# matchylabs/matchy

Hardware: AMD Instinct MI355X
Metric: log GB/s scanned (matchy match hot path, 100K IoCs) (higher is better)
Workload: dtype u8

## Files before the change

matchy_amd/csrc/device_common.h:

```cpp
#pragma once
#include <hip/hip_runtime.h>

#include "domain_prefilter.h"
#include "hashes.h"
#include "scan_types.h"

namespace mxy {

constexpr uint32_t C_B = 1, C_DIG = 2, C_DOT = 4, C_COLON = 8, C_AT = 16, C_LD = 32, C_NL = 64, C_TLD1 = 128;

constexpr uint64_t bnd_lo() {
    uint64_t m = 0;
    const int cs[] = {0x09, 0x0a, 0x0d, 0x20, 0x22, 0x27, 0x28, 0x29, 0x2c, 0x2f, 0x3a, 0x3b, 0x3c, 0x3d, 0x3e};
    for (int c : cs) m |= 1ull << c;
    return m;
}
constexpr uint64_t bnd_hi() {
    uint64_t m = 0;
    const int cs[] = {0x40, 0x5b, 0x5d, 0x7b, 0x7d};
    for (int c : cs) m |= 1ull << (c - 64);
    return m;
}
__device__ __forceinline__ bool d_is_boundary(uint32_t b) {
    if (b >= 128) return false;
    uint64_t m = b < 64 ? bnd_lo() : bnd_hi();
    return (m >> (b & 63)) & 1;
}
__device__ __forceinline__ bool d_is_digit(uint32_t b) { return b - '0' < 10u; }
__device__ __forceinline__ bool d_is_alpha(uint32_t b) { return (b | 0x20) - 'a' < 26u; }
__device__ __forceinline__ bool d_is_alnum(uint32_t b) { return d_is_digit(b) || d_is_alpha(b); }
__device__ __forceinline__ bool d_is_hex(uint32_t b) { return d_is_digit(b) || ((b | 0x20) - 'a' < 6u); }
__device__ __forceinline__ bool d_is_domain_char_fast(uint32_t b) { return d_is_alnum(b) || b == '-' || b == '.' || b >= 0x80; }
__device__ __forceinline__ bool d_is_domain_char(uint32_t b) { return d_is_alnum(b) || b == '-' || b == '.'; }
__device__ __forceinline__ bool d_is_email_local(uint32_t b) { return d_is_alnum(b) || b == '.' || b == '-' || b == '_' || b == '+'; }

__device__ __forceinline__ uint32_t class_of(uint32_t b) {
    uint32_t c = 0;
    if (d_is_boundary(b)) c |= C_B;
    if (d_is_digit(b)) c |= C_DIG;
    if (b == '.') c |= C_DOT;
    if (b == ':') c |= C_COLON;
    if (b == '@') c |= C_AT;
    if (d_is_alnum(b) || b >= 0x80) c |= C_LD;
    if (b == '\n') c |= C_NL;
    return c;
}

__device__ __forceinline__ uint32_t lane_id() { return __lane_id(); }
__device__ __forceinline__ uint64_t lanemask_lt() { return (1ull << lane_id()) - 1ull; }
__device__ __forceinline__ uint32_t mbcnt64_add(uint64_t m, uint32_t base) {
    return __builtin_amdgcn_mbcnt_hi((uint32_t)(m >> 32), __builtin_amdgcn_mbcnt_lo((uint32_t)m, base));
}
__device__ __forceinline__ uint32_t mbcnt64(uint64_t m) {
    return __builtin_amdgcn_mbcnt_hi((uint32_t)(m >> 32), __builtin_amdgcn_mbcnt_lo((uint32_t)m, 0u));
}

template <class T, uint32_t CHUNK>
struct ChunkWriter {
    static_assert(CHUNK >= 64, "one append can carry 64 entries");
    uint32_t base = 0xFFFFFFFFu;
    uint32_t used = 0;
    uint32_t total = 0;

    __device__ __forceinline__ void pad_rest(T* out, uint32_t cap, const T& sentinel) {
        if (base == 0xFFFFFFFFu) return;
        for (uint32_t k = used + lane_id(); k < CHUNK; k += 64)
            if (base + k < cap) out[base + k] = sentinel;
        used = CHUNK;
    }
    __device__ __forceinline__ void append(bool emit, const T& v, T* out, uint32_t cap, uint32_t* counter, const T& sentinel) {
        const uint64_t m = __ballot(emit);
        if (m == 0) return;
        const uint32_t n = (uint32_t)__popcll(m);
        if (base == 0xFFFFFFFFu || used + n > CHUNK) {
            pad_rest(out, cap, sentinel);
            uint32_t b = 0;
            if (lane_id() == 0) b = atomicAdd(counter, CHUNK);
            base = __builtin_amdgcn_readfirstlane(b);
            used = 0;
        }
        if (emit) {
            const uint32_t slot = base + used + (uint32_t)__popcll(m & lanemask_lt());
            if (slot < cap) out[slot] = v;
        }
        used += n;
        total += n;
    }
};

template <class T> __device__ __forceinline__ T list_sentinel();
template <> __device__ __forceinline__ Candidate list_sentinel<Candidate>() { return Candidate{0u, 0xFFFFFFFFu, 0u, 0u}; }
template <> __device__ __forceinline__ RareAnchor list_sentinel<RareAnchor>() { return RareAnchor{0xFFFFFFFFu, 0xFFu}; }
template <> __device__ __forceinline__ uint32_t list_sentinel<uint32_t>() { return 0xFFFFFFFFu; }
template <> __device__ __forceinline__ uint2 list_sentinel<uint2>() { return make_uint2(0xFFFFFFFFu, 0xFFu); }

template <class T, uint32_t CAP = 64>
struct BufferedWriter {
    T* buf;
    uint32_t cnt = 0;
    uint32_t total = 0;
    uint32_t base = 0xFFFFFFFFu, used = 0, ccap = 0, flushes = 0;
    __device__ __forceinline__ explicit BufferedWriter(T* lds) : buf(lds) {}
    __device__ __forceinline__ void pad_rest(T* out, uint32_t cap) {
        if (base == 0xFFFFFFFFu) return;
        for (uint32_t k = used + lane_id(); k < ccap; k += 64) if (base + k < cap) out[base + k] = list_sentinel<T>();
        used = ccap;
    }
// ... 285 lines not shown
```

matchy_amd/csrc/engine.cpp:

```cpp
#include "engine.h"
#include "batch_reader.h"
#include "distinct.h"
#include "extract_render_core.h"
#include "render_core.h"
#include "tally.h"
#include "unicode_lower.h"

#include <dlfcn.h>

#include <algorithm>
#include <chrono>
#include <cstdio>
#include <cstdlib>
#include <cstring>
#include <stdexcept>
#include <unordered_set>

#include "domain_prefilter.h"
#include "hashes.h"

namespace mxy {

void check_launch(const char* kernel) {
    const hipError_t e = hipGetLastError();
// ... 375 lines not shown
        for (const CpRange& r : lt.ignorable) ri.push_back(make_uint2(r.first, r.last));
        for (const CpRange& r : lt.cased) rc.push_back(make_uint2(r.first, r.last));
        lc_map.upload(m); lc_ign.upload(ri); lc_cased.upload(rc);
        view.lc_map = lc_map.p; view.lc_n = (uint32_t)lt.map.size();
        view.lc_ign = lc_ign.p; view.lc_n_ign = (uint32_t)ri.size();
        view.lc_cased = lc_cased.p; view.lc_n_cased = (uint32_t)rc.size();
        bytes_uploaded += m.size() * 4 + (ri.size() + rc.size()) * 8;
    }
    {
        std::vector<uint32_t> lo, go;
        if (img.has_literal) {
            if (!img.lit_data_offsets.empty()) lo = img.lit_data_offsets;
            else {
                uint32_t mx = 0;
                for (auto& kv : img.lit_data_map) mx = std::max(mx, kv.first + 1);
                lo.assign(mx, 0xFFFFFFFFu);
                for (auto& kv : img.lit_data_map) lo[kv.first] = kv.second;
            }
        }
        if (img.has_glob) {
            go.resize(img.pdm_count);
            if (img.pdm_count) memcpy(go.data(), img.bytes.data() + img.pdm_off, img.pdm_count * 4);
        }
        if (lo.empty()) lo.push_back(0xFFFFFFFFu);
        if (go.empty()) go.push_back(0);
        n_lit_offsets = img.has_literal ? (uint32_t)lo.size() : 0;
        n_glob_offsets = img.has_glob ? (uint32_t)img.pdm_count : 0;
        lit_offsets.upload(lo);
        glob_offsets.upload(go);
    }
    psl_slots.upload(psl.slots);
    psl_pool.upload(psl.pool);
    bloom.upload(psl.bloom);
    view.psl_slots = psl_slots.p; view.psl_mask = psl.mask; view.psl_pool = psl_pool.p; view.tld_bloom = bloom.p;
    view.max_tld_len = psl.max_tld_len;
    view.max_suffix_len = psl.max_suffix_len;
    tld_tab.upload(psl.tld_tab);
    view.tld_tab = tld_tab.p;
    tld_pfx.upload(psl.tld_pfx);
    view.tld_pfx = tld_pfx.p;
    for (int k = 0; k < 8; ++k) view.tld_first[k] = psl.tld_first[k];
    bytes_uploaded += psl.slots.size() * sizeof(PslSlot) + psl.pool.size() + psl.bloom.size() * 4;
}

Scanner::Scanner(std::shared_ptr<const DbImage> img, std::shared_ptr<DeviceDb> ddb, uint32_t extract_flags, uint32_t min_labels)
    : img_(std::move(img)), ddb_(std::move(ddb)), flags_(extract_flags), min_labels_(min_labels ? min_labels : 2) {
    MXY_HIP(hipSetDevice(ddb_->device));
    hipDeviceProp_t prop;
    MXY_HIP(hipGetDeviceProperties(&prop, ddb_->device));
    n_cu_ = prop.multiProcessorCount > 0 ? prop.multiProcessorCount : 256;
    counters_.alloc(MAX_SLICES);
    MXY_HIP(hipMemset(counters_.p, 0, sizeof(ScanCounters) * MAX_SLICES));
    counters_clean_ = true;
    host_slices_.alloc(MAX_SLICES);
    for (Event& e : ev_) e.create();
    ev_fork_.create(hipEventDisableTiming);
    ev_join_.create(hipEventDisableTiming);
    aux_stream_.create(hipStreamNonBlocking);
    ev_join2_.create(hipEventDisableTiming);
    aux2_stream_.create(hipStreamNonBlocking);
}

Scanner::~Scanner() = default;

void Scanner::set_unique(bool on) {
    if (on && !distinct_) {
        distinct_ = std::make_unique<DistinctSet>();
        if (getenv("MATCHY_AMD_TRACE")) { distinct_->set_profile(true); profile_ = true; }
    }
    unique_ = on;
}
void Scanner::reset_unique() {
    if (!distinct_) return;
    MXY_HIP(hipSetDevice(ddb_->device));
    distinct_->reset();
}
uint64_t Scanner::unique_count() const { return distinct_ ? distinct_->count() : 0; }

void Scanner::set_tally(bool on) {
    if (on && !tally_) tally_ = std::make_unique<HitTally>();
    tally_on_ = on;
}
void Scanner::reset_tally() {
    if (!tally_) return;
    MXY_HIP(hipSetDevice(ddb_->device));
    tally_->reset();
}
void Scanner::tally_top(size_t limit, std::vector<TallyEntry>& out) {
    out.clear();
    if (!tally_) return;
    MXY_HIP(hipSetDevice(ddb_->device));
    tally_->top(limit, out, nullptr);
}

void Scanner::Work::ensure(uint32_t len) {
    const size_t want_c = std::max<size_t>(4096, (size_t)len / 24);
    const size_t want_r = std::max<size_t>(1024, (size_t)len / 256);
    const size_t want_h = std::max<size_t>(1024, want_c / 4);
    if (cands.n < want_c) cands.alloc(want_c);
    if (hits.n < want_h) hits.alloc(want_h);
    if (ids.n < want_h) ids.alloc(want_h);
    if (cands_a.n < want_c) cands_a.alloc(want_c);
    if (cands_m.n < want_c / 8) cands_m.alloc(want_c / 8);
    if (cands_r.n < want_r) cands_r.alloc(want_r);
    if (cands_d.n < want_r) cands_d.alloc(want_r);
    if (rare.n < want_r) rare.alloc(want_r);
    if (rare_dom.n < want_r) rare_dom.alloc(want_r);
// ... 1207 lines not shown
```

matchy_amd/csrc/k_anchor.hip:

```cpp
#include "anchor_planes.h"
#include "device_shared.h"

namespace mxy {

constexpr int AW = 4;
constexpr int PRIO_BULK = 0, PRIO_CHAIN = 1, PRIO_DRAIN = 2;
constexpr uint32_t BLK_BYTES = AB_BLOCK;
constexpr uint32_t QCAP = 128;
constexpr uint32_t RAW_BYTES = 8192;
static_assert(SEG_ALIGN % RAW_BYTES == 0 && RAW_BYTES % BLK_BYTES == 0 && RAW_BYTES >= 3 * BLK_BYTES, "window wraps on block edges inside a segment");

constexpr uint32_t RAW_MIRROR = 64;
template <int N>
__device__ __forceinline__ void raw_read(const uint32_t* raw32, uint32_t a, uint32_t (&out)[N]) {
    static_assert(4 * (N + 1) <= RAW_MIRROR + 4, "read runs past the mirrored bytes");
    const uint32_t* q = raw32 + ((a & (RAW_BYTES - 1)) >> 2);
    const uint32_t sh = a & 3;
    uint32_t w[N + 1];
#pragma unroll
    for (int i = 0; i <= N; ++i) w[i] = q[i];
#pragma unroll
    for (int i = 0; i < N; ++i) out[i] = __builtin_amdgcn_alignbyte(w[i + 1], w[i], sh);
}

// ... 635 lines not shown
                    uint32_t cleft = cand;
                    while (__ballot(cleft != 0)) {
                        const bool mine = cleft != 0;
                        const uint32_t q = mine ? (uint32_t)__builtin_ctz(cleft) : 0u;
                        cleft &= cleft - 1;
                        const uint64_t Zq = (uint64_t)(uint32_t)__builtin_amdgcn_ds_bpermute((int)(4 * (q + 1)), zt) |
                                            ((uint64_t)(uint32_t)__builtin_amdgcn_ds_bpermute((int)(4 * (q + 17)), zt) << 32);
                        const uint64_t Zprev_row = (uint64_t)(uint32_t)__builtin_amdgcn_ds_bpermute((int)(4 * q), zt) |
                                                   ((uint64_t)(uint32_t)__builtin_amdgcn_ds_bpermute((int)(4 * (q + 16)), zt) << 32);
                        const uint64_t below = lane ? (Zq << (64 - lane)) : 0ull;
                        uint32_t run = lane ? (uint32_t)__clzll((long long)~below) : 0u;
                        run = min(run, lane);
                        bool too_long = false;
                        if (run == lane) {
                            const uint32_t r2 = ~Zprev_row ? (uint32_t)__clzll((long long)~Zprev_row) : 64u;
                            too_long = r2 == 64u;
                            run += r2;
                        }
                        const int32_t it = (int32_t)(64 * q + lane) - (int32_t)run - 1;
                        const uint32_t src_lane = (uint32_t)it & 63u;
                        const uint32_t wb_cur = (uint32_t)__shfl((int)Bcur, (int)src_lane);
                        const uint32_t wb_prev = (uint32_t)__shfl((int)Bprev, (int)src_lane);
                        const uint32_t rowbits = it >= 0 ? ((wb_cur >> (it >> 6)) & 0x01010101u) : ((wb_prev >> 7) & 0x01010101u);
                        const uint32_t hb = rowbits ? (31u - (uint32_t)__clz((int)rowbits)) >> 3 : 0u;
                        const int32_t s = (int32_t)blk + 4 * it + (int32_t)hb + 1;
                        const uint32_t mybits = (Bcur >> q) & 0x01010101u;
                        const uint32_t b0 = mybits ? ((uint32_t)__ffs((int)mybits) - 1u) >> 3 : 0u;
                        const uint32_t e = blk + AB_ROW_BYTES * q + lane_off + b0;
                        const uint32_t tl = e - (uint32_t)s;
                        const bool tok = mine && !too_long && rowbits != 0 &&
                                         ((tl >= 26 && tl <= 62) || tl == 64 || (tl >= 90 && tl <= 110) || tl == 128);
                        cw_tok.append(tok, make_uint2((uint32_t)s, (uint32_t)RARE_TOK | (tl << 8)));
                    }
                    tok_quiet = 0;
                } else if (tok_dense && ++tok_quiet >= TOK_DENSE_HOLD) {
                    tok_dense = false;
                }
                Bprev = Bcur;
            }
        }
        if (dt != dh) drain_dom(rdom, dh, dt, dt - dh, true, cx, cw_dom);
        if (v4t != v4h) drain_v4<INL>(rv4, v4h, v4t, v4t - v4h, true, cx, pend, cw_cand, vl);
    }
    commit_v4<INL>(pend, cx, cw_cand, vl);
    if constexpr (INL) v4_lookup_flush(vl);
    cw_misc.finish();
    cw_tok.finish();
    if (cw_dom.next == 0xFFFFFFFFu && cold_tok()->dom_static) {
        cw_dom.next = (blockIdx.x * 4u + (threadIdx.x >> 6)) * cold_tok()->dom_static;
        cw_dom.left = cold_tok()->dom_static;
    }
    cw_dom.pad_rest(p.dom_list, p.dom_cap);
    cw_cand.finish(p.cands_a, p.cand_a_cap, &p.counters->n_cand_a, Candidate{0u, 0xFFFFFFFFu, 0u, 0u});
    {
        uint32_t nv = pend.n_valid;
#pragma unroll
        for (int off = 32; off > 0; off >>= 1) nv += __shfl_down(nv, off);
        if (lane == 0 && nv) atomicAdd(&cold_tok()->counters->cand_true, nv);
    }
    unsigned long long lines = nl_count;
#pragma unroll
    for (int off = 32; off > 0; off >>= 1) lines += __shfl_down(lines, off);
    if (lane == 0 && lines) atomicAdd(&cold_tok()->counters->lines, lines);
}

int anchor_blocks_per_cu() {
    int n = 0;
    const hipError_t e = hipOccupancyMaxActiveBlocksPerMultiprocessor(&n, k_anchor<true, true>, AW * 64, 0);
    if (e != hipSuccess || n < 1) n = 3;
    return n;
}

void launch_anchor(const TokParams& p, const DevDb& db, int grid, hipStream_t stream) {
    const bool all = (p.flags & EX_ALL) == EX_ALL && !anchor_tl_wide(db);
    if (all && p.inline_v4) hipLaunchKernelGGL((k_anchor<true, true>), dim3(grid), dim3(AW * 64), 0, stream, p, db);
    else if (all) hipLaunchKernelGGL((k_anchor<true, false>), dim3(grid), dim3(AW * 64), 0, stream, p, db);
    else if (p.inline_v4) hipLaunchKernelGGL((k_anchor<false, true>), dim3(grid), dim3(AW * 64), 0, stream, p, db);
    else hipLaunchKernelGGL((k_anchor<false, false>), dim3(grid), dim3(AW * 64), 0, stream, p, db);
    check_launch("launch_anchor");
}

}
```

matchy_amd/csrc/lookup_kernels.hip:

```cpp
#include <hip/hip_runtime.h>

#include <cstdlib>

#include "hashes.h"
#include "scan_types.h"

#include "device_shared.h"

namespace mxy {


__device__ __forceinline__ uint32_t d_utf8_decode(const uint8_t* s, uint32_t& cp) {
    const uint32_t c = s[0];
    if (c < 0x80) { cp = c; return 1; }
    if (c < 0xE0) { cp = ((c & 0x1Fu) << 6) | (s[1] & 0x3Fu); return 2; }
    if (c < 0xF0) { cp = ((c & 0x0Fu) << 12) | ((s[1] & 0x3Fu) << 6) | (s[2] & 0x3Fu); return 3; }
    cp = ((c & 0x07u) << 18) | ((s[1] & 0x3Fu) << 12) | ((s[2] & 0x3Fu) << 6) | (s[3] & 0x3Fu);
    return 4;
}
__device__ bool d_cp_in_ranges(const uint2* r, uint32_t n, uint32_t cp) {
    uint32_t lo = 0, hi = n;
    while (lo < hi) { const uint32_t mid = (lo + hi) >> 1; if (r[mid].y < cp) lo = mid + 1; else hi = mid; }
    return lo < n && r[lo].x <= cp;
}
// ... 540 lines not shown
            uint32_t type = c.len_type >> 24, tl = c.len_type & 0xFFFFFF;
            const uint8_t* text = p.log + c.start;
            h.cand = i; h.start = c.start; h.len_type = c.len_type;
            if (type == IT_IPV4) {
                uint32_t off, pfx;
                if (db.has_ip && trie_v4(db, c.v4, off, pfx)) { h.kind = 2; h.a = off; h.prefix_len = (uint8_t)pfx; emit = true; }
            } else if (type == IT_IPV6) {
                uint16_t seg[8];
                uint32_t off, pfx;
                if (db.has_ip && d_parse_ipv6(text, tl, seg) && trie_v6(db, seg, off, pfx)) { h.kind = 2; h.a = off; h.prefix_len = (uint8_t)pfx; emit = true; }
            } else {
                const bool alnum_tok = type == IT_MD5 || type == IT_SHA1 || type == IT_SHA256 || type == IT_SHA384 || type == IT_SHA512 ||
                                       type == IT_BITCOIN || type == IT_ETHEREUM || type == IT_MONERO;
                if (!db.ac_alnum && alnum_tok) c.pad = CAND_NO_GLOB;
                if (!GLOB && p.ac_filter && p.early_glob && c.pad == CAND_GLOB) {
                } else if (!GLOB && p.ac_filter && (c.pad == CAND_GLOB || (c.pad != CAND_NO_GLOB && (defer_unwalked || ac_touches_output(db, dv, text, tl))))) defer = true;
                else {
                    uint32_t pid = 0xFFFFFFFFu;
                    if (db.has_literal) { uint32_t q; if (lit_lookup(db, text, tl, q)) pid = q; }
                    if constexpr (GLOB) {
                        GlobSetList rs{globs};
                        StarStackFixed stk;
                        glob_find_all(db, dv, text_stage(p.log, p.len, c.start, tl, twin + threadIdx.x * GLOB_WIN_WORDS), outq + threadIdx.x * GLOB_OUTQ, rs, stk);
                        ng = rs.n;
                        spill = rs.over;
                    }
                    if (!spill && (pid != 0xFFFFFFFFu || ng)) { h.kind = 3; h.a = pid; h.n_globs = (uint16_t)ng; emit = true; }
                }
            }
        }
        if (p.direct && !GLOB) {
            if (emit) { pend[pn] = PendRec{h.start, h.len_type, h.a, (uint32_t)h.kind | ((uint32_t)h.prefix_len << 8)}; ++pn; }
            if (__ballot(pn == PEND_RECS)) { pack_pending(p.pk, pn, pend); pn = 0; }
        } else if (p.direct) {
            pack_record(p.pk, emit, h, GLOB ? globs : nullptr);
        } else {
            if (GLOB && emit && ng) {
                uint32_t io = atomicAdd(&p.counters->n_ids, ng);
                h.ids_off = io;
                for (uint32_t k = 0; k < ng; ++k) if (io + k < p.ids_cap) p.ids[io + k] = globs[k];
            }
            cw.append(emit, h, p.hits, p.hit_cap, &p.counters->n_hits, SH);
        }
        if (!GLOB && p.ac_filter) ww.append(defer, i, p.glob_work, p.glob_work_cap, &p.counters->n_glob_work);
        if (GLOB && spill) {
            const uint32_t q = atomicAdd(&p.counters->n_spill, 1u);
            if (q < p.spill_cap) p.spill[q] = i | (p.spill_tag << 31);
        }
    }
    __shared__ uint32_t wg_slots[12];
    if (p.direct && !GLOB) pack_pending<PEND_RECS, true>(p.pk, pn, pend, wg_slots);
    cw.pad_rest(p.hits, p.hit_cap, SH);
    if (!GLOB && p.ac_filter) ww.flush(p.glob_work, p.glob_work_cap, &p.counters->n_glob_work);
    if (lane_id() == 0 && cw.total) atomicAdd(&p.counters->hits_true, cw.total);
    if (p.arrive_chain) {
        __syncthreads();
        if (threadIdx.x == 0) {
            __threadfence_system();
            if (atomicAdd(&p.arrive->arrive_wgs[p.arrive_chain - 1], 1u) == gridDim.x - 1) atomicAdd(&p.arrive->chains_done, 1u);
        }
    }
}

constexpr int SPILL_THREADS = 64;
__global__ __launch_bounds__(SPILL_THREADS) void k_lookup_spill(LookupParams p, DevDb db) {
    __shared__ uint8_t cls[256];
    __shared__ uint32_t rows[DFA_LDS_ENTRIES_GLOB];
    __shared__ uint64_t twin[SPILL_THREADS * GLOB_WIN_WORDS];
    __shared__ uint32_t outq[SPILL_THREADS * GLOB_OUTQ];
    const DfaView dv = dfa_stage<DFA_LDS_ENTRIES_GLOB>(db, cls, rows);
    __syncthreads();
    const uint32_t n = min(p.counters->n_spill, p.spill_cap);
    const uint32_t stride = gridDim.x * blockDim.x, tid = blockIdx.x * blockDim.x + threadIdx.x;
    const uint32_t bit_words = (db.pattern_count + 31) / 32;
    uint32_t* bits = p.spill_scratch + (size_t)tid * p.spill_words;
    ChunkWriter<Hit, HIT_CHUNK> cw;
    Hit SH{};
    SH.kind = 0xFF;
    for (uint32_t base = blockIdx.x * blockDim.x; base < n; base += stride) {
        const uint32_t k = base + threadIdx.x;
        Hit h{};
        bool emit = false;
        if (k < n) {
            const uint32_t tagged = p.spill[k], i = tagged & 0x7FFFFFFFu;
            const bool alt = (tagged >> 31) != 0;
            const Candidate c = alt ? (p.cands_alt && i < p.cand_alt_cap ? p.cands_alt[i] : Candidate{0, 0xFFFFFFFFu, 0, 0})
                                    : (i < p.cand_cap ? p.cands[i] : Candidate{0, 0xFFFFFFFFu, 0, 0});
            if (c.len_type != 0xFFFFFFFFu) {
                const uint32_t tl = c.len_type & 0xFFFFFF;
                h.cand = i; h.start = c.start; h.len_type = c.len_type;
                uint32_t pid = 0xFFFFFFFFu;
                if (db.has_literal) { uint32_t q; if (lit_lookup(db, p.log + c.start, tl, q)) pid = q; }
                for (uint32_t w = 0; w < bit_words; ++w) bits[w] = 0;
                GlobSetBitmap rs{bits, db.pattern_count};
                StarStackMem stk{bits + bit_words, (p.spill_words - bit_words) / 2};
                glob_find_all(db, dv, text_stage(p.log, p.len, c.start, tl, twin + threadIdx.x * GLOB_WIN_WORDS), outq + threadIdx.x * GLOB_OUTQ, rs, stk);
                uint32_t ng = rs.n;
                if (rs.over || ng > 0xFFFFu) { atomicOr(&p.counters->error, 1u); ng = 0; }
                if (ng) {
                    const uint32_t io = atomicAdd(&p.counters->n_ids, ng);
                    h.ids_off = io;
                    uint32_t o = io;
                    for (uint32_t w = 0; w < bit_words; ++w)
                        for (uint32_t m = bits[w]; m; m &= m - 1, ++o)
                            if (o < p.ids_cap) p.ids[o] = 32 * w + (uint32_t)__builtin_ctz(m);
                }
                if (pid != 0xFFFFFFFFu || ng) { h.kind = 3; h.a = pid; h.n_globs = (uint16_t)ng; emit = true; }
            }
        }
        if (p.direct) pack_record(p.pk, emit, h, nullptr);
        else cw.append(emit, h, p.hits, p.hit_cap, &p.counters->n_hits, SH);
    }
    cw.pad_rest(p.hits, p.hit_cap, SH);
    if (lane_id() == 0 && cw.total) atomicAdd(&p.counters->hits_true, cw.total);
}

template <uint32_t NREC>
__global__ __launch_bounds__(256) void k_lookup_ip(LookupParams p, DevDb db) {
    __shared__ __attribute__((aligned(16))) PendRec pend_lds[256 * NREC];
    PendRec* pend = pend_lds + threadIdx.x * NREC;
    uint32_t pn = 0;
    const uint32_t n = min(*p.n_in, p.cand_cap);
    const uint32_t stride = gridDim.x * blockDim.x;
    for (uint32_t base = blockIdx.x * blockDim.x; base < n; base += stride) {
        const uint32_t i = base + threadIdx.x;
        Candidate c{0, 0xFFFFFFFFu, 0, 0};
        if (i < n) c = p.cands[i];
        if (c.len_type != 0xFFFFFFFFu && (c.len_type >> 24) == IT_IPV4) {
            uint32_t off, pfx;
            if (db.has_ip && trie_v4(db, c.v4, off, pfx)) { pend[pn] = PendRec{c.start, c.len_type, off, 2u | (pfx << 8)}; ++pn; }
        }
        if (__ballot(pn == NREC)) { pack_pending<NREC>(p.pk, pn, pend); pn = 0; }
    }
    __shared__ uint32_t wg_slots[12];
    pack_pending<NREC, true>(p.pk, pn, pend, wg_slots);
}
void launch_lookup_ip(const LookupParams& p, const DevDb& db, int grid, bool dense, hipStream_t stream) {
    if (dense) hipLaunchKernelGGL(k_lookup_ip<8>, dim3(grid), dim3(256), 0, stream, p, db);
    else hipLaunchKernelGGL(k_lookup_ip<2>, dim3(grid), dim3(256), 0, stream, p, db);
    check_launch("launch_lookup_ip");
}
void launch_lookup(const LookupParams& p_in, const DevDb& db, int grid, hipStream_t stream) {
    LookupParams p = p_in;
    p.ac_filter = 0; p.from_work = 0;
    const size_t lean_lds = db.dfa ? (size_t)DFA_LDS_ENTRIES * 4 : 0;
    if (!db.has_glob) {
        hipLaunchKernelGGL(k_lookup<false>, dim3(grid), dim3(256), lean_lds, stream, p, db);
    } else if (db.dfa && db.wild_count == 0 && p.glob_work && grid > 1) {
        p.ac_filter = 1;
        const uint32_t arrive_chain = p.arrive_chain;
        p.arrive_chain = 0;
        hipLaunchKernelGGL(k_lookup<false>, dim3(grid), dim3(256), lean_lds, stream, p, db);
        p.arrive_chain = arrive_chain;
        p.ac_filter = 0; p.from_work = 1;
        hipLaunchKernelGGL(k_lookup<true>, dim3(grid), dim3(256), 0, stream, p, db);
    } else {
        hipLaunchKernelGGL(k_lookup<true>, dim3(grid), dim3(256), 0, stream, p, db);
    }
    check_launch("launch_lookup");
}
void launch_lookup_early_glob(const LookupParams& p_in, const DevDb& db, int grid, hipStream_t stream) {
    LookupParams p = p_in;
    p.ac_filter = 0; p.from_work = 1;
    hipLaunchKernelGGL(k_lookup<true>, dim3(grid), dim3(256), 0, stream, p, db);
    check_launch("launch_lookup_early_glob");
}
__global__ __launch_bounds__(256) void k_finish(ScanCounters* dev, ScanCounters* host, uint32_t n_words, uint32_t expect_chains, unsigned long long poll_ticks,
                                                uint32_t next_n_dom) {
    uint32_t* d = reinterpret_cast<uint32_t*>(dev);
    uint32_t* h = reinterpret_cast<uint32_t*>(host);
    __shared__ uint32_t gave_up;
    if (threadIdx.x == 0) gave_up = 0;
    if (expect_chains) {
        if (threadIdx.x == 0) {
            const unsigned long long t0 = wall_clock64();
            if (poll_ticks == 0) gave_up = 1;
            else while (__hip_atomic_load(&dev->chains_done, __ATOMIC_ACQUIRE, __HIP_MEMORY_SCOPE_AGENT) < expect_chains) {
                if (wall_clock64() - t0 > poll_ticks) { gave_up = 1; break; }
                __builtin_amdgcn_s_sleep(8);
            }
        }
        __syncthreads();
        __threadfence();
    } else {
        __syncthreads();
    }
    const bool keep = gave_up != 0;
    for (uint32_t i = threadIdx.x; i < n_words; i += blockDim.x) {
        h[i] = d[i];
        if (!keep) d[i] = 0;
    }
    __syncthreads();
    if (!keep && threadIdx.x == 0 && next_n_dom) dev->n_dom = next_n_dom;
    if (keep && threadIdx.x == 0) host->error |= 8u;
    __threadfence_system();
}
void launch_finish(ScanCounters* dev, ScanCounters* host_pinned, int n_blocks, uint32_t expect_chains, uint32_t next_n_dom, hipStream_t stream) {
    static const unsigned long long poll_ticks = getenv("MATCHY_AMD_FINISH_POLL_US") ? strtoull(getenv("MATCHY_AMD_FINISH_POLL_US"), nullptr, 10) * 100ull : 200000000ull;
    hipLaunchKernelGGL(k_finish, dim3(1), dim3(256), 0, stream, dev, host_pinned, (uint32_t)(n_blocks * sizeof(ScanCounters) / 4), expect_chains, poll_ticks, next_n_dom);
    check_launch("launch_finish");
}
void launch_lookup_spill(const LookupParams& p, const DevDb& db, hipStream_t stream) {
    hipLaunchKernelGGL(k_lookup_spill, dim3(p.spill_blocks), dim3(SPILL_THREADS), 0, stream, p, db);
    check_launch("launch_lookup_spill");
}
uint32_t spill_threads() { return SPILL_THREADS; }

}
```

matchy_amd/csrc/scan_types.h:

```cpp
#pragma once
#include <hip/hip_runtime.h>

#include <cstdint>

namespace mxy {

enum ItemType : uint8_t {
    IT_DOMAIN = 0, IT_EMAIL = 1, IT_IPV4 = 2, IT_IPV6 = 3, IT_MD5 = 4, IT_SHA1 = 5, IT_SHA256 = 6,
    IT_SHA384 = 7, IT_SHA512 = 8, IT_BITCOIN = 9, IT_ETHEREUM = 10, IT_MONERO = 11, IT_COUNT = 12
};
enum ExtractFlags : uint32_t {
    EX_DOMAINS = 1, EX_EMAILS = 2, EX_IPV4 = 4, EX_IPV6 = 8, EX_HASHES = 16, EX_BITCOIN = 32, EX_ETHEREUM = 64,
    EX_MONERO = 128, EX_ALL = 255
};

struct Candidate {
    uint32_t start;
    uint32_t len_type;
    uint32_t v4;
    uint32_t pad;
};
constexpr uint32_t CAND_NO_GLOB = 1, CAND_GLOB = 2;

enum RareKind : uint32_t { RARE_V6 = 0, RARE_AT = 1, RARE_TOK = 2, HEAVY_B58 = 3, HEAVY_BECH32 = 4, HEAVY_ETH = 5, HEAVY_XMR = 6, RARE_DOM = 7 };
// ... 31 lines not shown
    const LitSlot* lit_slots;
    uint32_t lit_mask;
    uint32_t has_literal;
    const uint32_t* lit_bm;
    uint32_t lit_bm_mask;
    const uint8_t* lit_pool;
    uint32_t lit_pool_size;
    uint32_t lit_max_len;
    const uint8_t* pg;
    uint32_t pg_len;
    uint32_t has_glob;
    uint32_t ac_start, ac_size;
    uint32_t patterns_off, pattern_count;
    uint32_t wild_off, wild_count;
    uint32_t glob_seg_off;
    uint32_t glob_max_segs;
    const uint32_t* dfa;
    const uint8_t* dfa_cls;
    const uint32_t* dfa_node;
    uint32_t dfa_k;
    uint32_t dfa_states;
    const uint32_t* sfx_bm;
    uint32_t sfx_mask;
    uint32_t sfx_first;
    uint32_t sfx_dots;
    const uint32_t* lit2pat_off;
    const uint32_t* lit2pat;
    uint32_t n_ac_lits;
    uint32_t ac_alnum;
    const PslSlot* psl_slots;
    uint32_t psl_mask;
    const uint8_t* psl_pool;
    const uint32_t* tld_bloom;
    uint32_t max_tld_len;
    uint32_t max_suffix_len;
    const uint2* tld_tab;
    uint32_t tld_first[8];
    uint32_t ci;
    const uint32_t* lc_map;
    uint32_t lc_n;
    const uint2* lc_ign;
    uint32_t lc_n_ign;
    const uint2* lc_cased;
    uint32_t lc_n_cased;
    const uint2* tld_pfx;
};

constexpr uint32_t DFA_LDS_ENTRIES = 8192;
constexpr uint32_t DFA_LDS_ENTRIES_GLOB = 2048;
constexpr uint32_t DFA_LDS_ENTRIES_VAL = 2048;
constexpr uint32_t TLD_BLOOM_BITS = 32768;
constexpr uint32_t TLD_BLOOM_WORDS = TLD_BLOOM_BITS / 32;

struct ScanCounters {
    alignas(128) unsigned long long lines;
    uint32_t cand_true;
    uint32_t hits_true;
    uint32_t error;
    uint32_t reserved0;
    alignas(128) uint32_t n_cand;
    alignas(128) uint32_t n_cand_a;
    alignas(128) uint32_t n_cand_m;
    uint32_t n_cand_d;
    uint32_t n_cand_r;
    alignas(128) uint32_t n_dom;
    alignas(128) uint32_t n_rare;
    alignas(128) uint32_t n_rare_dom;
    alignas(128) uint32_t n_tok;
    alignas(128) uint32_t n_heavy;
    alignas(128) uint32_t n_hits;
    uint32_t n_ids;
    alignas(128) uint32_t n_final;
    uint32_t n_final_ids;
    uint32_t n_c4;
    alignas(128) uint32_t chains_done;
    uint32_t arrive_wgs[3];
    alignas(128) uint32_t n_glob_work;
    uint32_t n_glob_work_d;
    uint32_t n_spill;
};

struct FinalHit {
    uint32_t start;
    uint32_t len_type;
    uint32_t value;
    uint8_t kind, prefix_len;
    uint16_t n_ids;
};

struct PackParams {
    const Hit* hits;
    uint32_t hit_cap;
    const uint32_t* ids;
    uint32_t ids_cap;
    const uint32_t* lit_offsets;
    uint32_t n_lit;
    const uint32_t* glob_offsets;
    uint32_t n_glob;
    FinalHit* out;
    uint32_t out_cap;
    uint32_t* out_ids;
    long long* out_offs;
    uint32_t out_ids_cap;
    FinalHit* host_out;
    uint32_t host_cap;
    uint32_t* host_ids;
    long long* host_offs;
    uint32_t host_ids_cap;
    uint2* c4_out;
    uint2* host_c4;
    uint32_t c4_cap, host_c4_cap;
    ScanCounters* counters;
};

constexpr uint32_t C4_DATA_BITS = 22;
__host__ __device__ inline uint2 c4_pack(uint32_t start, uint32_t len, uint32_t data_off, uint32_t prefix) {
    return make_uint2(start, data_off | ((len - 7u) << C4_DATA_BITS) | (prefix << (C4_DATA_BITS + 4)));
}

struct TokParams {
    const uint8_t* log;
    uint32_t len;
    uint32_t flags;
    uint32_t min_labels;
    uint32_t debug;
    uint32_t filter_v4;
    uint32_t filter_lit;
    uint32_t filter_ac;
    uint32_t n_segs;
    uint32_t seg_bytes;
    uint32_t seg_base;
    uint32_t scan_end;
// ... 76 lines not shown
```

matchy_amd/csrc/validate_kernels.hip:

```cpp
#include <hip/hip_runtime.h>

#include <cstdlib>

#include "hashes.h"
#include "scan_types.h"

#include "device_shared.h"
#include "domain_planes.h"

namespace mxy {


struct BackReader {
    const uint8_t* p;
    uint32_t pos;
    uint32_t cb;
    uint32_t k;
    uint64_t cur, nxt;
    __device__ __forceinline__ static uint64_t load8(const uint8_t* a) { uint64_t v; __builtin_memcpy(&v, a, 8); return v; }
    __device__ __forceinline__ void init(const uint8_t* base, uint32_t q) {
        p = base; pos = q; cb = 0; k = 0; cur = 0; nxt = 0;
        if (q >= 16) { cb = q - 8; k = 8; cur = load8(p + cb); nxt = load8(p + cb - 8); }
    }
    __device__ __forceinline__ uint32_t next() {
// ... 861 lines not shown
                                uint32_t m = M;
                                for (uint32_t j = 1; j < d; ++j) m &= ~(m ? (0x80000000u >> __builtin_clz(m)) : 0u);
                                if (m) {
                                    const uint32_t kk = 31u - (uint32_t)__builtin_clz(m), sl = n - kk;
                                    if (sl >= 3) {
                                        const uint32_t o2 = o + kk, j0 = o2 >> 2, s2 = o2 & 3;
                                        uint32_t w2[9];
#pragma unroll
                                        for (int k = 0; k < 9; ++k) w2[k] = (j0 + k) < 8 ? sb[(j0 + k) & 7] : 0u;
                                        uint64_t l2[4];
#pragma unroll
                                        for (int k = 0; k < 4; ++k)
                                            l2[k] = (uint64_t)__builtin_amdgcn_alignbyte(w2[2 * k + 1], w2[2 * k], s2) |
                                                    ((uint64_t)__builtin_amdgcn_alignbyte(w2[2 * k + 2], w2[2 * k + 1], s2) << 32);
                                        if (db.ci) {
#pragma unroll
                                            for (int k = 0; k < 4; ++k) l2[k] = ascii_lower8(l2[k]);
                                        }
                                        const uint32_t b2 = name_hash31(l2[0], l2[1], l2[2], l2[3], sl) & db.sfx_mask;
                                        pend_sw[q] = db.sfx_bm[b2 >> 5];
                                        pend_sb[q] = b2 & 31;
                                    }
                                }
                            }
                        }
                    }
                    if constexpr (AC) {
                        uint32_t st = 0, any = 0;
#pragma unroll
                        for (int k = 0; k < 31; ++k) {
                            const uint32_t c = dcls[(uint32_t)(ln[k >> 3] >> (8 * (k & 7))) & 0xFF];
                            if ((uint32_t)k < n) {
                                const uint32_t t = st < dv.lds_states ? drows[st * db.dfa_k + c] : db.dfa[(size_t)st * db.dfa_k + c];
                                st = t & 0x7FFFFFFFu;
                                any |= t;
                            }
                        }
                        pend_over = (any >> 31) != 0;
                        if (pend_over) { pend_word = 0xFFFFFFFFu; pend_bit = 0; }
                    }
                }
            }
        }
        sw.append(slow, RareAnchor{cur.j & 0x7FFFFFFFu, (uint32_t)RARE_DOM}, p.rare_dom, p.rare_dom_cap, &p.counters->n_rare_dom);
        cur = nxt;
    }
    emit_pending();
    if constexpr (AC || SFX) cw.flush_then(p.cands, p.cand_cap, p.n_cand, queue_glob);
    else cw.flush(p.cands, p.cand_cap, p.n_cand);
    cw_dense.pad_rest(p.cands, p.cand_cap, SC);
    sw.flush(p.rare_dom, p.rare_dom_cap, &p.counters->n_rare_dom);
#pragma unroll
    for (int off = 32; off > 0; off >>= 1) n_valid += __shfl_down(n_valid, off);
    if (lane_id() == 0 && n_valid) atomicAdd(&p.counters->cand_true, n_valid);
}

__device__ __forceinline__ bool lit_bm_may_hit(const DevDb& db, const LogView& lg, uint32_t s, uint32_t n, bool ascii) {
    uint64_t l[4] = {0, 0, 0, 0};
    if (s + 32 <= lg.len) {
#pragma unroll
        for (int k = 0; k < 4; ++k) __builtin_memcpy(&l[k], lg.p + s + 8 * k, 8);
    } else {
        for (uint32_t k = 0; k < 32 && s + k < lg.len; ++k) l[k >> 3] |= (uint64_t)lg.p[s + k] << (8 * (k & 7));
    }
    if (db.ci) {
        if (!ascii) {
            if (n > 32) return true;
            uint64_t high = 0;
#pragma unroll
            for (int k = 0; k < 4; ++k) {
                const int rem = (int)n - 8 * k;
                const uint64_t m = rem >= 8 ? ~0ull : (rem <= 0 ? 0ull : ((1ull << (8 * rem)) - 1ull));
                high |= l[k] & m & 0x8080808080808080ull;
            }
            if (high) return true;
        }
#pragma unroll
        for (int k = 0; k < 4; ++k) l[k] = ascii_lower8(l[k]);
    }
    const uint32_t b = name_hash31(l[0], l[1], l[2], l[3], n) & db.lit_bm_mask;
    return ((db.lit_bm[b >> 5] >> (b & 31)) & 1u) != 0;
}

template <uint32_t VM>
__global__ __launch_bounds__(256) void k_validate(TokParams p, DevDb db) {
    constexpr bool MISC = (VM & 1u) != 0, DOM = (VM & 2u) != 0, TOK = (VM & 4u) != 0;
    __shared__ uint32_t bloom[DOM ? TLD_BLOOM_WORDS : 1];
    constexpr bool TLD_LDS = DOM && (MISC || TOK);
    __shared__ uint2 tldtab[TLD_LDS ? (1u << TLD_TAB_BITS) : 1];
    const uint2* const tldtab_p = TLD_LDS ? tldtab : db.tld_tab;
    constexpr uint32_t WIN = MISC ? 80 : 64;
    constexpr uint32_t WIN_BACK = WIN - (MISC ? 32 : 16);
    __shared__ __attribute__((aligned(16))) uint8_t winbuf[(MISC || DOM) ? 256 * WIN : 16];
    if constexpr (DOM && !MISC && !TOK) {
        if (blockIdx.x * blockDim.x >= min(p.counters->n_rare_dom, p.rare_dom_cap)) return;
    }
    if constexpr (TOK && !MISC && !DOM) {
        if (blockIdx.x * blockDim.x >= min(p.counters->n_tok, p.tok_cap)) return;
    }
    if constexpr (DOM) {
        for (uint32_t i = threadIdx.x; i < TLD_BLOOM_WORDS; i += blockDim.x) bloom[i] = db.tld_bloom[i];
        if constexpr (TLD_LDS) for (uint32_t i = threadIdx.x; i < (1u << TLD_TAB_BITS); i += blockDim.x) tldtab[i] = db.tld_tab[i];
        __syncthreads();
    }
    LogView lg{p.log, p.len};
    __shared__ Candidate wb_cand[4][64];
    BufferedWriter<Candidate> cw(wb_cand[threadIdx.x >> 6]);
// ... 214 lines not shown
                    if (rw != 2) { todo = false; dr = rw == 1 ? WALK_YES : WALK_NO; ds = s2; de = e2; }
                }
            }
            const bool inner = todo && ra.pos >= WIN_BACK && ra.pos + (WIN - WIN_BACK) <= lg.len;
            if (__ballot(inner)) {
                if (inner) fill_window(ra.pos - WIN_BACK);
                __builtin_amdgcn_wave_barrier();
                if (inner) {
                    const LogView wv{win, WIN};
                    bool edge = false;
                    uint32_t s2 = 0, e2 = 0;
                    const int rw = val_domain(wv, db, bloom, tldtab_p, p.min_labels, WIN_BACK, s2, e2, nullptr, &edge);
                    if (!edge) { todo = false; dr = rw; ds = s2 + (ra.pos - WIN_BACK); de = e2 + (ra.pos - WIN_BACK); }
                }
            }
            if (todo) {
                const uint32_t a0 = ra.pos & ~127u;
                uint32_t t0 = lg.p[a0], t1 = a0 >= 128 ? lg.p[a0 - 128] : 0u;
                asm volatile("" ::"v"(t0), "v"(t1));
                dr = val_domain(lg, db, bloom, tldtab_p, p.min_labels, ra.pos, ds, de, &dl);
            }
        }
        for (uint64_t lm = __ballot(dr == WALK_LONG); lm; lm &= lm - 1) {
            const int src = __ffsll((long long)lm) - 1;
            WalkState st;
            st.pos = (uint32_t)__shfl((int)dl.st.pos, src); st.cur = (uint32_t)__shfl((int)dl.st.cur, src);
            st.last_c = (uint32_t)__shfl((int)dl.st.last_c, src); st.labels = (uint32_t)__shfl((int)dl.st.labels, src);
            st.high = __shfl((int)dl.st.high, src) != 0; st.bad = __shfl((int)dl.st.bad, src) != 0; st.found = __shfl((int)dl.st.found, src) != 0;
            coop_domain_skip(lg, st);
            if ((int)lane_id() == src) dl.st = st;
        }
        bool need_u8 = false;
        if (dr == WALK_LONG) dr = val_domain_resume(lg, db, p.min_labels, dl, ds, de, need_u8) ? WALK_YES : WALK_NO;
        for (uint64_t lm = __ballot(dr == WALK_YES && need_u8); lm; lm &= lm - 1) {
            const int src = __ffsll((long long)lm) - 1;
            const uint32_t us = (uint32_t)__shfl((int)ds, src), ue = (uint32_t)__shfl((int)de, src);
            const bool good = coop_valid_utf8(lg.p + us, ue - us);
            if ((int)lane_id() == src && !good) dr = WALK_NO;
        }
        if (dr == WALK_YES) {
            if (de - ds > 0xFFFFFFu) atomicOr(&p.counters->error, 4u);
            c.start = ds; c.len_type = (de - ds) | ((uint32_t)IT_DOMAIN << 24); emit = true;
        }
        if (lit_only && emit) {
            const uint32_t ty = c.len_type >> 24;
            if ((ty == IT_EMAIL || ty == IT_DOMAIN) && !lit_bm_may_hit(db, lg, c.start, c.len_type & 0xFFFFFFu, ty == IT_EMAIL)) { emit = false; ++unlisted; }
        }
        cw.append(emit, c, p.cands, p.cand_cap, p.n_cand);
    }
    }
    cw.flush(p.cands, p.cand_cap, p.n_cand);
#pragma unroll
    for (int off = 32; off > 0; off >>= 1) unlisted += __shfl_down(unlisted, off);
    if (lane_id() == 0 && cw.total + unlisted) atomicAdd(&p.counters->cand_true, cw.total + unlisted);
}

__global__ __launch_bounds__(64) void k_rare(TokParams p, DevDb db) {
    __shared__ __attribute__((aligned(16))) uint8_t tokbuf[64][112];
    __shared__ __attribute__((aligned(16))) uint8_t decbuf[64][96];
    LogView lg{p.log, p.len};
    __shared__ Candidate wb_cand[64];
    BufferedWriter<Candidate> cw(wb_cand);
    const uint32_t n = min(p.counters->n_heavy, p.heavy_cap);
    uint8_t* tb = tokbuf[threadIdx.x];
    uint8_t* dec = decbuf[threadIdx.x];
    for (uint32_t base = blockIdx.x * 64; base < n; base += gridDim.x * 64) {
        const uint32_t i = base + threadIdx.x;
        RareAnchor ra{0, 0xFF};
        if (i < n) ra = p.heavy[i];
        const uint32_t kind = ra.len_kind & 0xFF, tl = ra.len_kind >> 8;
        bool em = false;
        Candidate ct{0, 0, 0, 0};
        if (kind != 0xFF && tl <= 110) {
            for (uint32_t k = 0; k < tl; k += 16) {
                if (ra.pos + k + 16 <= lg.len) {
                    uint4 v;
                    __builtin_memcpy(&v, lg.p + ra.pos + k, 16);
                    *reinterpret_cast<uint4*>(tb + k) = v;
                } else {
                    for (uint32_t b = k; b < tl; ++b) tb[b] = lg.p[ra.pos + b];
                }
            }
            int ty = -1;
            if (kind == HEAVY_BECH32) { if (val_btc_bech32(tb, tl)) ty = IT_BITCOIN; }
            else if (kind == HEAVY_B58) { if (val_btc_base58(tb, tl, dec)) ty = IT_BITCOIN; }
            else if (kind == HEAVY_ETH) { if (val_eth(tb, dec)) ty = IT_ETHEREUM; }
            else if (kind == HEAVY_XMR) { if (val_monero(tb, tl, dec)) ty = IT_MONERO; }
            if (ty >= 0) { ct.start = ra.pos; ct.len_type = tl | ((uint32_t)ty << 24); em = true; }
        }
        cw.append(em, ct, p.cands, p.cand_cap, p.n_cand);
    }
    cw.flush(p.cands, p.cand_cap, p.n_cand);
    if (lane_id() == 0 && cw.total) atomicAdd(&p.counters->cand_true, cw.total);
}

int validate_blocks_per_cu(bool ac) {
    int n = 0;
    const hipError_t e = ac ? hipOccupancyMaxActiveBlocksPerMultiprocessor(&n, k_validate_dom<1>, 256, 0)
                            : hipOccupancyMaxActiveBlocksPerMultiprocessor(&n, k_validate_dom<0>, 256, 0);
    if (e != hipSuccess || n < 1) n = ac ? 3 : 4;
    return n;
}
void launch_validate_dom(const TokParams& p, const DevDb& db, int grid, hipStream_t stream) {
    if (!(p.flags & EX_DOMAINS)) return;
    if (p.filter_ac && db.sfx_bm) hipLaunchKernelGGL(k_validate_dom<2>, dim3(grid), dim3(256), 0, stream, p, db);
    else if (p.filter_ac) hipLaunchKernelGGL(k_validate_dom<1>, dim3(grid), dim3(256), 0, stream, p, db);
    else hipLaunchKernelGGL(k_validate_dom<0>, dim3(grid), dim3(256), 0, stream, p, db);
    check_launch("launch_validate_dom");
}
void launch_validate_misc(const TokParams& p, const DevDb& db, int grid, hipStream_t stream) {
    if (p.vmode == 5u) hipLaunchKernelGGL(k_validate<5u>, dim3(grid), dim3(256), 0, stream, p, db);
    else if (p.vmode == 4u) hipLaunchKernelGGL(k_validate<4u>, dim3(grid), dim3(256), 0, stream, p, db);
    else if (p.vmode == 1u) hipLaunchKernelGGL(k_validate<1u>, dim3(grid), dim3(256), 0, stream, p, db);
    else if (p.vmode == 2u) hipLaunchKernelGGL(k_validate<2u>, dim3(grid), dim3(256), 0, stream, p, db);
    else hipLaunchKernelGGL(k_validate<7u>, dim3(grid), dim3(256), 0, stream, p, db);
    check_launch("launch_validate_misc");
}
void launch_rare(const TokParams& p, const DevDb& db, int grid, hipStream_t stream) {
    hipLaunchKernelGGL(k_rare, dim3(grid), dim3(64), 0, stream, p, db);
    check_launch("launch_rare");
}

}
```

Before: 2392.

## Stripe statistic counters and aggregate per workgroup to cut global atomic contention

```diff
diff --git a/matchy_amd/csrc/device_common.h b/matchy_amd/csrc/device_common.h
--- a/matchy_amd/csrc/device_common.h
+++ b/matchy_amd/csrc/device_common.h
@@ -53,6 +53,21 @@
 }
 __device__ __forceinline__ uint32_t mbcnt64(uint64_t m) {
     return __builtin_amdgcn_mbcnt_hi((uint32_t)(m >> 32), __builtin_amdgcn_mbcnt_lo((uint32_t)m, 0u));
+}
+
+__device__ __forceinline__ StatStripe* stat_stripe(ScanCounters* c) { return &c->stripes[blockIdx.x % STAT_STRIPES]; }
+
+__device__ __forceinline__ void wg_stat_add(uint32_t* xch, uint32_t stride, uint32_t wave, ScanCounters* counters, unsigned long long lines, uint32_t cand_true) {
+    if (lane_id() == 0) { uint32_t* m = xch + wave * stride; m[0] = (uint32_t)lines; m[1] = (uint32_t)(lines >> 32); m[2] = cand_true; }
+    __syncthreads();
+    if (threadIdx.x == 0) {
+        unsigned long long l = 0;
+        uint32_t c = 0;
+        for (uint32_t w = 0; w < blockDim.x / 64; ++w) { const uint32_t* m = xch + w * stride; l += m[0] | ((unsigned long long)m[1] << 32); c += m[2]; }
+        StatStripe* const s = stat_stripe(counters);
+        if (l) atomicAdd(&s->lines, l);
+        if (c) atomicAdd(&s->cand_true, c);
+    }
 }
 
 template <class T, uint32_t CHUNK>
diff --git a/matchy_amd/csrc/engine.cpp b/matchy_amd/csrc/engine.cpp
--- a/matchy_amd/csrc/engine.cpp
+++ b/matchy_amd/csrc/engine.cpp
@@ -451,7 +451,9 @@
     counters_.alloc(MAX_SLICES);
     MXY_HIP(hipMemset(counters_.p, 0, sizeof(ScanCounters) * MAX_SLICES));
     counters_clean_ = true;
+    static_assert(MAX_SLICES <= MAX_COUNTER_BLOCKS, "k_finish sums the stripes of every slice's block in LDS");
     host_slices_.alloc(MAX_SLICES);
+    memset(host_slices_.p, 0, sizeof(ScanCounters) * MAX_SLICES);
     for (Event& e : ev_) e.create();
     ev_fork_.create(hipEventDisableTiming);
     ev_join_.create(hipEventDisableTiming);
diff --git a/matchy_amd/csrc/k_anchor.hip b/matchy_amd/csrc/k_anchor.hip
--- a/matchy_amd/csrc/k_anchor.hip
+++ b/matchy_amd/csrc/k_anchor.hip
@@ -711,16 +711,13 @@
     }
     cw_dom.pad_rest(p.dom_list, p.dom_cap);
     cw_cand.finish(p.cands_a, p.cand_a_cap, &p.counters->n_cand_a, Candidate{0u, 0xFFFFFFFFu, 0u, 0u});
-    {
-        uint32_t nv = pend.n_valid;
-#pragma unroll
-        for (int off = 32; off > 0; off >>= 1) nv += __shfl_down(nv, off);
-        if (lane == 0 && nv) atomicAdd(&cold_tok()->counters->cand_true, nv);
-    }
+    uint32_t nv = pend.n_valid;
+#pragma unroll
+    for (int off = 32; off > 0; off >>= 1) nv += __shfl_down(nv, off);
     unsigned long long lines = nl_count;
 #pragma unroll
     for (int off = 32; off > 0; off >>= 1) lines += __shfl_down(lines, off);
-    if (lane == 0 && lines) atomicAdd(&cold_tok()->counters->lines, lines);
+    wg_stat_add(q_v4[0], QCAP, wave, cold_tok()->counters, lines, nv);
 }
 
 int anchor_blocks_per_cu() {
diff --git a/matchy_amd/csrc/lookup_kernels.hip b/matchy_amd/csrc/lookup_kernels.hip
--- a/matchy_amd/csrc/lookup_kernels.hip
+++ b/matchy_amd/csrc/lookup_kernels.hip
@@ -616,7 +616,7 @@
     if (p.direct && !GLOB) pack_pending<PEND_RECS, true>(p.pk, pn, pend, wg_slots);
     cw.pad_rest(p.hits, p.hit_cap, SH);
     if (!GLOB && p.ac_filter) ww.flush(p.glob_work, p.glob_work_cap, &p.counters->n_glob_work);
-    if (lane_id() == 0 && cw.total) atomicAdd(&p.counters->hits_true, cw.total);
+    if (lane_id() == 0 && cw.total) atomicAdd(&stat_stripe(p.counters)->hits_true, cw.total);
     if (p.arrive_chain) {
         __syncthreads();
         if (threadIdx.x == 0) {
@@ -676,7 +676,7 @@
         else cw.append(emit, h, p.hits, p.hit_cap, &p.counters->n_hits, SH);
     }
     cw.pad_rest(p.hits, p.hit_cap, SH);
-    if (lane_id() == 0 && cw.total) atomicAdd(&p.counters->hits_true, cw.total);
+    if (lane_id() == 0 && cw.total) atomicAdd(&stat_stripe(p.counters)->hits_true, cw.total);
 }
 
 template <uint32_t NREC>
@@ -750,8 +750,30 @@
         __syncthreads();
     }
     const bool keep = gave_up != 0;
+    constexpr uint32_t BW = sizeof(ScanCounters) / 4, HW = offsetof(ScanCounters, stripes) / 4;
+    static_assert(offsetof(ScanCounters, lines) == 0 && offsetof(ScanCounters, cand_true) == 8 && offsetof(ScanCounters, hits_true) == 12, "words 0..3 of a block are its totals");
+    __shared__ unsigned long long tot_lines[MAX_COUNTER_BLOCKS];
+    __shared__ uint32_t tot_cand[MAX_COUNTER_BLOCKS], tot_hits[MAX_COUNTER_BLOCKS];
+    const uint32_t n_blocks = n_words / BW;
+    if (threadIdx.x < n_blocks) { tot_lines[threadIdx.x] = 0; tot_cand[threadIdx.x] = 0; tot_hits[threadIdx.x] = 0; }
+    __syncthreads();
+    if (threadIdx.x < n_blocks) {
+        atomicAdd(&tot_lines[threadIdx.x], dev[threadIdx.x].lines); atomicAdd(&tot_cand[threadIdx.x], dev[threadIdx.x].cand_true); atomicAdd(&tot_hits[threadIdx.x], dev[threadIdx.x].hits_true);
+    }
+    for (uint32_t i = threadIdx.x; i < n_blocks * STAT_STRIPES; i += blockDim.x) {
+        const StatStripe s = dev[i / STAT_STRIPES].stripes[i % STAT_STRIPES];
+        if (s.lines) atomicAdd(&tot_lines[i / STAT_STRIPES], s.lines);
+        if (s.cand_true) atomicAdd(&tot_cand[i / STAT_STRIPES], s.cand_true);
+        if (s.hits_true) atomicAdd(&tot_hits[i / STAT_STRIPES], s.hits_true);
+    }
+    __syncthreads();
     for (uint32_t i = threadIdx.x; i < n_words; i += blockDim.x) {
-        h[i] = d[i];
+        const uint32_t b = i / BW, w = i % BW;
+        if (w < HW) {
+            uint32_t v = d[i];
+            if (w < 4) v = w == 0 ? (uint32_t)tot_lines[b] : w == 1 ? (uint32_t)(tot_lines[b] >> 32) : w == 2 ? tot_cand[b] : tot_hits[b];
+            h[i] = v;
+        }
         if (!keep) d[i] = 0;
     }
     __syncthreads();
diff --git a/matchy_amd/csrc/scan_types.h b/matchy_amd/csrc/scan_types.h
--- a/matchy_amd/csrc/scan_types.h
+++ b/matchy_amd/csrc/scan_types.h
@@ -107,6 +107,13 @@
 constexpr uint32_t TLD_BLOOM_BITS = 32768;
 constexpr uint32_t TLD_BLOOM_WORDS = TLD_BLOOM_BITS / 32;
 
+constexpr uint32_t STAT_STRIPES = 32;
+constexpr int MAX_COUNTER_BLOCKS = 8;
+struct StatStripe {
+    alignas(128) unsigned long long lines;
+    uint32_t cand_true;
+    uint32_t hits_true;
+};
 struct ScanCounters {
     alignas(128) unsigned long long lines;
     uint32_t cand_true;
@@ -133,6 +140,7 @@
     alignas(128) uint32_t n_glob_work;
     uint32_t n_glob_work_d;
     uint32_t n_spill;
+    StatStripe stripes[STAT_STRIPES];
 };
 
 struct FinalHit {
diff --git a/matchy_amd/csrc/validate_kernels.hip b/matchy_amd/csrc/validate_kernels.hip
--- a/matchy_amd/csrc/validate_kernels.hip
+++ b/matchy_amd/csrc/validate_kernels.hip
@@ -937,7 +937,7 @@
     sw.flush(p.rare_dom, p.rare_dom_cap, &p.counters->n_rare_dom);
 #pragma unroll
     for (int off = 32; off > 0; off >>= 1) n_valid += __shfl_down(n_valid, off);
-    if (lane_id() == 0 && n_valid) atomicAdd(&p.counters->cand_true, n_valid);
+    wg_stat_add(&strbuf[0][0], 64 * 8, threadIdx.x >> 6, p.counters, 0ull, n_valid);
 }
 
 __device__ __forceinline__ bool lit_bm_may_hit(const DevDb& db, const LogView& lg, uint32_t s, uint32_t n, bool ascii) {
@@ -1258,7 +1258,7 @@
     cw.flush(p.cands, p.cand_cap, p.n_cand);
 #pragma unroll
     for (int off = 32; off > 0; off >>= 1) unlisted += __shfl_down(unlisted, off);
-    if (lane_id() == 0 && cw.total + unlisted) atomicAdd(&p.counters->cand_true, cw.total + unlisted);
+    wg_stat_add(reinterpret_cast<uint32_t*>(&wb_cand[0][0]), 64 * (uint32_t)(sizeof(Candidate) / 4), threadIdx.x >> 6, p.counters, 0ull, cw.total + unlisted);
 }
 
 __global__ __launch_bounds__(64) void k_rare(TokParams p, DevDb db) {
@@ -1297,7 +1297,7 @@
         cw.append(em, ct, p.cands, p.cand_cap, p.n_cand);
     }
     cw.flush(p.cands, p.cand_cap, p.n_cand);
-    if (lane_id() == 0 && cw.total) atomicAdd(&p.counters->cand_true, cw.total);
+    if (lane_id() == 0 && cw.total) atomicAdd(&stat_stripe(p.counters)->cand_true, cw.total);
 }
 
 int validate_blocks_per_cu(bool ac) {
```

Result: no change. 2404 (median of 3 runs) (+0.5%).
